# loop-Z/omniisaacgymenvs_loop

Measured on AMD Instinct MI355X. Metric: env-steps/sec USV_CaptureXY at 1/2/4/8 MI355X; wall-clock to reward=30, higher is better.
Workload: dtype fp32

## Files before the change

### omniisaacgymenvs_loop_amd/csrc/ppo.hip

```cpp
#include <cstdlib>
#include <cstring>
#include <type_traits>

#include "usv_device.h"

USV_PROBE_DEFINE(ppo)
USV_PROBE_DEFINE(pol)
USV_PROBE_DEFINE(red)

namespace {

constexpr int NIN = PPO_NIN, NH = PPO_NH, NA = PPO_NA;
constexpr int RB = 32;
constexpr int TB = 256;
constexpr int XS = 35;
constexpr int HS = 129;
constexpr int NPART = PPO_NPARAM + 8;
constexpr int NPART_PAD = (NPART + 3) & ~3;
constexpr int P_LOSS = PPO_NPARAM;
constexpr float kLog2Pi = 1.8378770664093453f;

typedef float f32x16 __attribute__((ext_vector_type(16)));
typedef unsigned int u32x4_t __attribute__((ext_vector_type(4)));

// ... 797 lines not shown
#pragma unroll
      for (int u = 0; u < 8; ++u) xv[u] = obs[(size_t)min(r0 + u * nl, bnd - 1) * NIN + col];
#pragma unroll
      for (int u = 0; u < 8; ++u)
        if (r0 + u * nl < bnd) {
          const double x = xv[u];
          s += x; s2 += x * x;
        }
    }
    acc[0][col][lane_r] = s;
    acc[1][col][lane_r] = s2;
  }
  __syncthreads();
  if (tid < NIN) {
    double t = 0, t2 = 0;
    for (int l = 0; l < nl; ++l) { t += acc[0][tid][l]; t2 += acc[1][tid][l]; }
    double *o = part + ((size_t)mb * OM_CH + ch) * 2 * NIN;
    o[tid] = t;
    o[NIN + tid] = t2;
  }
}

constexpr int RS_TB = 256, RS_U = 8;
__global__ __launch_bounds__(RS_TB) void k_obs_rms_seq(ppo_cfg_t c, const double *__restrict__ part, int nmb,
                                                       double *obs_rms, double *seq) {
  const double rows = (double)c.minibatch;
  for (int q = threadIdx.x; q < nmb * NIN; q += RS_TB) {
    const int mb = q / NIN, k = q % NIN;
    double sa = 0, sb = 0;
#pragma unroll
    for (int ch = 0; ch < OM_CH; ++ch) {
      const double *o = part + ((size_t)mb * OM_CH + ch) * 2 * NIN;
      sa += o[k];
      sb += o[NIN + k];
    }
    const double bmean = sa / rows;
    seq[(size_t)mb * 2 * NIN + k] = bmean;
    seq[(size_t)mb * 2 * NIN + NIN + k] = (sb - rows * bmean * bmean) / (rows - 1.0);
  }
  __syncthreads();
  const int k = threadIdx.x;
  if (k < NIN) {
    double mean = obs_rms[k], var = obs_rms[NIN + k], count = obs_rms[2 * NIN];
    for (int mb0 = 0; mb0 < nmb; mb0 += RS_U) {
      double bm[RS_U], bv[RS_U];
#pragma unroll
      for (int u = 0; u < RS_U; ++u) {
        const int mb = min(mb0 + u, nmb - 1);
        bm[u] = seq[(size_t)mb * 2 * NIN + k];
        bv[u] = seq[(size_t)mb * 2 * NIN + NIN + k];
      }
#pragma unroll
      for (int u = 0; u < RS_U; ++u) {
        if (mb0 + u >= nmb) break;
        const double tot = count + rows;
        const double delta = bm[u] - mean;
        const double M2 = var * count + bv[u] * rows + delta * delta * count * rows / tot;
        mean = mean + delta * rows / tot;
        var = M2 / tot;
        count = tot;
        seq[(size_t)(mb0 + u) * 2 * NIN + k] = mean;
        seq[(size_t)(mb0 + u) * 2 * NIN + NIN + k] = var;
      }
    }
    obs_rms[k] = mean;
    obs_rms[NIN + k] = var;
    if (k == 0) obs_rms[2 * NIN] = count;
  }
}

constexpr int GTB = 512;

#ifndef USV_RD_P
#define USV_RD_P 128
#endif
typedef float f32x4v __attribute__((ext_vector_type(4)));
constexpr int RD_TB = 512, RD_P = USV_RD_P;
constexpr int RD_L = RD_P / 4;
constexpr int RD_G = (RD_TB / RD_L);
constexpr int RD_KB = 16;
constexpr int RED_BLOCKS = (PPO_NPARAM + 5 + RD_P - 1) / RD_P;
static_assert(RD_P % 4 == 0 && 64 % RD_L == 0 && RD_P <= RD_TB, "reduce geometry");
static_assert(RED_BLOCKS <= 256, "chunk squares: one per thread of waves 0-3");
constexpr int W2IMG_FLOATS = (NH * HS + 3) & ~3;
constexpr int W2IMG_OFF = (PPO_NPARAM + 8 + RED_BLOCKS + 3) & ~3;
constexpr int W2IMG_PIECES = W2IMG_FLOATS / 256;
constexpr int W2IMG_LAST_LANES = W2IMG_FLOATS % 256 / 4;
static_assert(W2IMG_FLOATS == NH * HS && W2IMG_PIECES % 8 == 0 && W2IMG_LAST_LANES > 0 && W2IMG_LAST_LANES < 64,
              "W2 image: the copy covers s.w2 exactly, 8 waves x whole pieces + one partial piece");

struct AdamBanks {
  const float *P0, *m0, *v0;
  float *P1, *m1, *v1;
};
struct AdamK {
  float step_size, bc2s;
};
__device__ __forceinline__ AdamK adam_consts(const ppo_cfg_t &c, float lr, float step) {
  const double bc1 = 1.0 - pow((double)c.adam_b1, (double)step);
  const double bc2 = 1.0 - pow((double)c.adam_b2, (double)step);
  return {(float)((double)lr / bc1), (float)sqrt(bc2)};
}
__device__ __forceinline__ void adam_one(const ppo_cfg_t &c, const AdamK &k, float g, float p_old, float m_old,
                                         float v_old, float &pn, float &mn, float &vn) {
  if (c.weight_decay != 0.f) g = g + c.weight_decay * p_old;
  mn = m_old + (1.0f - c.adam_b1) * (g - m_old);
  vn = v_old * c.adam_b2 + (1.0f - c.adam_b2) * g * g;
  const float denom = sqrtf(vn) / k.bc2s + c.adam_eps;
  pn = p_old - k.step_size * (mn / denom);
}
__device__ __forceinline__ float clip_coef(const ppo_cfg_t &c, float total_norm) {
  float coef = 1.0f;
  if (c.truncate_grads) {
    coef = c.grad_norm / (total_norm + 1e-6f);
    coef = fminf(coef, 1.0f);
  }
  return coef;
}
__device__ __forceinline__ AdamK adam_consts_tagged(const ppo_cfg_t &c, float lr, float step, float t_ss,
                                                    float t_bc, float t_step, float t_lr) {
  if (t_step == step && t_lr == lr) return {t_ss, t_bc};
  return adam_consts(c, lr, step);
}
struct OptNext {
  float nl, kl_keep, step;
  AdamK nk;
};
template <class OptIn>
__device__ __forceinline__ OptNext opt_next(const ppo_cfg_t &c, const OptIn &opt_in, float kl) {
  const float lr = opt_in[0];
  float nl = lr, kl_keep = opt_in[2];
  if (c.lr_adaptive) {
    if (kl > 2.0f * c.kl_threshold) nl = fmaxf(lr / 1.5f, c.lr_min);
    if (kl < 0.5f * c.kl_threshold) nl = fminf(lr * 1.5f, c.lr_max);
    kl_keep = kl;
  }
  const float step = opt_in[1] + 1.0f;
  return {nl, kl_keep, step, adam_consts(c, nl, step + 1.0f)};
}
__device__ __forceinline__ void opt_store(const ppo_cfg_t &c, const OptNext &x, float *opt_out, float total_norm,
                                          float kl, float *kl_out) {
  if (c.lr_adaptive && kl_out) *kl_out = kl;
  opt_out[0] = x.nl;
  opt_out[1] = x.step;
  opt_out[2] = x.kl_keep;
  opt_out[3] = total_norm;
  opt_out[4] = x.nk.step_size;
  opt_out[5] = x.nk.bc2s;
  opt_out[6] = x.step + 1.0f;
  opt_out[7] = x.nl;
}

struct ChainIn {
  const float *P_prev, *m_prev, *v_prev;
  float *P_cur, *m_cur, *v_cur;
  const float *grad;
  const float *opt_prev;
  float *opt_cur;
  float *kl_out;
  uint32_t *dp_clock;
  int fold_skip;
  float gscale;
};

constexpr int XG = XS;
constexpr int GX = ((RB * XG + GTB - 1) / GTB) * GTB;
struct GradSmem {
  alignas(16) float w2[NH * HS];
  float w1[NH * XG];
  float x[GX];
  float h1[RB * HS];
  float h2[RB * HS];
  float xch[4][16][64];
  float out[RB * 4];
  float g[RB * 4];
  float hg[4][4][NH];
  float b1[NH];
  float tail[TAIL + 1];
  float nrm[4];
  int fold[2];
};

constexpr int S_W2 = 0, S_W1 = NH * NH, S_SIG = S_W1 + NH * 32, S_B1 = S_SIG + 2, S_TAIL = S_B1 + NH,
              S_W1C = S_TAIL + TAIL, S_END = S_W1C + NH;
static_assert(S_END == PPO_NPARAM && S_W1 % 4 == 0 && NIN == 33, "partial slot layout");
__device__ __forceinline__ int tail_slot(int param) { return S_TAIL + param - PPO_OFF_B2; }
__device__ __forceinline__ int acc_slot(int base, int tile, int a, int lane) { return base + ((tile * 4 + a) * 64 + lane) * 4; }
__device__ __forceinline__ int param_of_slot(int s) {
  if (s < S_W1) {
    const int tile = s >> 10, a = (s >> 8) & 3, lane = (s >> 2) & 63, q = 4 * a + (s & 3);
    const int n = 32 * (tile >> 2) + crow(q, lane >> 5), k = 32 * (tile & 3) + (lane & 31);
    return PPO_OFF_W2 + n * NH + k;
  }
  if (s < S_SIG) {
    const int t = s - S_W1, tile = t >> 10, a = (t >> 8) & 3, lane = (t >> 2) & 63, q = 4 * a + (t & 3);
    const int n = 32 * tile + crow(q, lane >> 5), k = lane & 31;
    return PPO_OFF_W1 + n * NIN + k;
  }
  if (s < S_B1) return PPO_OFF_SIGMA + (s - S_SIG);
  if (s < S_TAIL) return PPO_OFF_B1 + (s - S_B1);
  if (s < S_W1C) return PPO_OFF_B2 + (s - S_TAIL);
  if (s < S_END) return PPO_OFF_W1 + (s - S_W1C) * NIN + (NIN - 1);
  return -1;
}

struct RowIn {
  float act0, act1, nlp, val, ret, adv, mu0, mu1, sg0, sg1;
};

#ifndef USV_PART_AUX
#define USV_PART_AUX 2
#endif
template <int kAux, bool kCM>
struct PartOutT {
  __amdgpu_buffer_rsrc_t r;
  uint32_t cs;
  __device__ __forceinline__ uint32_t off(int idx) const {
    if constexpr (kCM) return (uint32_t)(idx / RD_P) * cs + (uint32_t)(idx % RD_P) * 4u;
    else return (uint32_t)idx * 4u;
  }
  __device__ __forceinline__ void operator()(int idx, float v) const {
    __builtin_amdgcn_raw_buffer_store_b32(__builtin_bit_cast(uint32_t, v), r, off(idx), 0, kAux);
  }
  __device__ __forceinline__ void x4(int idx, float a, float b, float c, float d) const {
    const u32x4_t v = {__builtin_bit_cast(uint32_t, a), __builtin_bit_cast(uint32_t, b), __builtin_bit_cast(uint32_t, c),
                       __builtin_bit_cast(uint32_t, d)};
    __builtin_amdgcn_raw_buffer_store_b128(v, r, off(idx), 0, kAux);
  }
};
constexpr int AUX_SC1 = 16;

constexpr int FOLD_G = 8;
static_assert(RD_G >= FOLD_G, "k_reduce_partials(fold = 1) reads one group row per row group");
constexpr int FOLD_MAX_M = 32;
constexpr int FOLD_CTL_STRIDE = 64;
constexpr uint64_t FOLD_WAIT_TICKS = 10000;
__host__ __device__ constexpr size_t part_body_floats(int nblk) {
  return (size_t)nblk * RED_BLOCKS * RD_P > (size_t)(nblk + FOLD_G) * NPART_PAD ? (size_t)nblk * RED_BLOCKS * RD_P
                                                                                 : (size_t)(nblk + FOLD_G) * NPART_PAD;
}
__device__ __forceinline__ uint32_t *fold_ctl(float *partials, int nblk) {
  return reinterpret_cast<uint32_t *>(partials + part_body_floats(nblk));
}
__device__ __forceinline__ const uint32_t *fold_ctl(const float *partials, int nblk) {
  return reinterpret_cast<const uint32_t *>(partials + part_body_floats(nblk));
}
__device__ __forceinline__ f32x4v ld4_sc1(__amdgpu_buffer_rsrc_t r, uint32_t byte_off) {
  return __builtin_bit_cast(f32x4v, __builtin_amdgcn_raw_buffer_load_b128(r, byte_off, 0, AUX_SC1));
}

__device__ __forceinline__ void lds_dma16(const float *src, uint32_t lds_dst) {
  uint32_t keep;
  __asm__ volatile("s_mov_b32 %0, m0\n\ts_mov_b32 m0, %2\n\ts_nop 0\n\tglobal_load_lds_dwordx4 %1, off\n\t"
                   "s_mov_b32 m0, %0"
                   : "=&s"(keep)
                   : "v"(src), "s"(lds_dst)
                   : "memory");
}

__device__ __forceinline__ void redo_step(const ppo_cfg_t &c, const ChainIn &ch, const float (&op)[8], float coef,
                                          float scale, GradSmem &s, float &ls0, float &ls1) {
  const AdamK ak = adam_consts_tagged(c, op[0], op[1] + 1.0f, op[4], op[5], op[6], op[7]);
  for (int q = threadIdx.x; q < PPO_NPARAM; q += GTB) {
    float pn, mn, vn;
    adam_one(c, ak, ch.grad[q] * scale * coef, ch.P_prev[q], ch.m_prev[q], ch.v_prev[q], pn, mn, vn);
    if ((q / GTB) % gridDim.x == blockIdx.x) {
      ch.P_cur[q] = pn; ch.m_cur[q] = mn; ch.v_cur[q] = vn;
    }
    if (q >= PPO_OFF_B2) {
      s.tail[q - PPO_OFF_B2] = pn;
    } else if (q >= PPO_OFF_W2) {
      const int e = q - PPO_OFF_W2;
      s.w2[(e / NH) * HS + e % NH] = pn;
    } else if (q >= PPO_OFF_B1) {
      s.b1[q - PPO_OFF_B1] = pn;
    } else if (q >= PPO_OFF_W1) {
      const int e = q - PPO_OFF_W1;
      s.w1[(e / NIN) * XG + e % NIN] = pn;
    }
  }
  float pn, mn, vn;
  adam_one(c, ak, ch.grad[PPO_OFF_SIGMA] * scale * coef, ch.P_prev[PPO_OFF_SIGMA], ch.m_prev[PPO_OFF_SIGMA],
           ch.v_prev[PPO_OFF_SIGMA], pn, mn, vn);
  ls0 = pn;
  adam_one(c, ak, ch.grad[PPO_OFF_SIGMA + 1] * scale * coef, ch.P_prev[PPO_OFF_SIGMA + 1],
           ch.m_prev[PPO_OFF_SIGMA + 1], ch.v_prev[PPO_OFF_SIGMA + 1], pn, mn, vn);
  ls1 = pn;
}

constexpr int APN_TB = 256;
__device__ __forceinline__ float apply_norm_part(const float *__restrict__ grad_in, float grad_scale, int tid) {
  constexpr int N4 = PPO_NPARAM / 4, U = (N4 + APN_TB - 1) / APN_TB;
  const float4 *g4 = reinterpret_cast<const float4 *>(grad_in);
  float4 gv[U];
#pragma unroll
  for (int u = 0; u < U; ++u) gv[u] = g4[min(tid + u * APN_TB, N4 - 1)];
  float ss = 0.f;
#pragma unroll
  for (int u = 0; u < U; ++u) {
    if (tid + u * APN_TB >= N4) continue;
    const float x = gv[u].x * grad_scale, y = gv[u].y * grad_scale;
    const float z = gv[u].z * grad_scale, w = gv[u].w * grad_scale;
    ss = fmaf(x, x, ss); ss = fmaf(y, y, ss); ss = fmaf(z, z, ss); ss = fmaf(w, w, ss);
  }
  for (int r = 4 * N4 + tid; r < PPO_NPARAM; r += APN_TB) {
    const float g = grad_in[r] * grad_scale;
    ss = fmaf(g, g, ss);
  }
  return ss;
}

template <bool kBf, bool kChain, bool kFold, bool kColl = false>
__device__ __forceinline__ void mb_grad8w(const ppo_cfg_t &c, const ChainIn &ch, const float *__restrict__ P,
                                          const double *__restrict__ obs_rms, int row0,
                                          const float *__restrict__ e_obs, const float *__restrict__ e_act,
                                          const float *__restrict__ e_nlp, const float *__restrict__ e_val,
                                          const float *__restrict__ e_ret, const float *__restrict__ e_adv,
                                          float *e_mu, float *e_sigma, float *partials, GradSmem &s) {
  const int tid = threadIdx.x, lane = tid & 63, w = tid >> 6;
  const int i = lane & 31, h = lane >> 5;
  const int kh = w >> 2, cb = w & 3, n0 = 32 * cb;
  const int rb0 = row0 + blockIdx.x * RB;
  const float invB = 1.0f / (float)c.minibatch;
  USV_PHASE(ppo, 0);
  if (ch.dp_clock && blockIdx.x == 0 && tid == 0) *ch.dp_clock += 1u;
  constexpr int NW1G = (NH * XG + GTB - 1) / GTB, NTLG = (TAIL + GTB - 1) / GTB, NW2F = NH * NH / GTB;
  static_assert(NH * NH % GTB == 0, "staging trip counts");
  constexpr bool kImg = kChain && !kColl && !kFold;
  float w2f[kImg ? 1 : NW2F];
  float w1r[NW1G], tlr[NTLG];
  float ov = 0.f;
  if constexpr (kChain) ov = lane < 8 ? ch.opt_prev[lane] : ch.grad[PPO_NPARAM];
  {
#pragma unroll
    for (int u = 0; u < NW1G; ++u) {
      const int q = min(tid + u * GTB, NH * XG - 1), j = q / XG, k = q % XG;
      w1r[u] = P[PPO_OFF_W1 + j * NIN + min(k, NIN - 1)];
    }
#pragma unroll
    for (int u = 0; u < NTLG; ++u) tlr[u] = P[PPO_OFF_B2 + min(tid + u * GTB, TAIL - 1)];
  }
  const float b1r = P[PPO_OFF_B1 + (tid & (NH - 1))];
  float lsv;
  if constexpr (!kImg) lsv = P[PPO_OFF_SIGMA + (lane & 1)];
  float lsig0 = 0.f, lsig1 = 0.f;
  float csq = 0.f;
  if constexpr (kChain) csq = ch.grad[PPO_NPARAM + 8 + min(tid, RED_BLOCKS - 1)];
  RowIn ri;
  const auto load_rows = [&] {
    const size_t row = (size_t)rb0 + (lane & (RB - 1));
    ri.act0 = e_act[row * 2]; ri.act1 = e_act[row * 2 + 1];
    ri.nlp = e_nlp[row]; ri.adv = e_adv[row];
    ri.val = e_val[row]; ri.ret = e_ret[row];
    ri.mu0 = e_mu[row * 2]; ri.mu1 = e_mu[row * 2 + 1];
    ri.sg0 = e_sigma[row * 2]; ri.sg1 = e_sigma[row * 2 + 1];
  };
  if constexpr (!kImg) load_rows();
  constexpr int NU = (RB * XG + GTB - 1) / GTB;
  float xo[NU];
  double mu[NU], var[NU];
#pragma unroll
  for (int u = 0; u < NU; ++u) {
    const int q = min(tid + u * GTB, RB * XG - 1), r = q / XG, kc = min(q % XG, NIN - 1);
    xo[u] = e_obs[(size_t)(rb0 + r) * NIN + kc];
    mu[u] = obs_rms[kc];
    var[u] = obs_rms[NIN + kc];
  }
  if constexpr (kImg) {
    lsv = P[PPO_OFF_SIGMA + (lane & 1)];
    load_rows();
    const int wu = __builtin_amdgcn_readfirstlane(w);
    const uint32_t w2lds = (uint32_t)(uintptr_t)(__attribute__((address_space(3))) float *)s.w2;
    const float *img = ch.grad + W2IMG_OFF + lane * 4;
    if (wu == GTB / 64 - 1 && lane < W2IMG_LAST_LANES)
      lds_dma16(img + W2IMG_PIECES * 256, w2lds + W2IMG_PIECES * 1024);
#pragma unroll
    for (int u = 0; u < W2IMG_PIECES / (GTB / 64); ++u) {
      const int pc = wu + (GTB / 64) * u;
      lds_dma16(img + pc * 256, w2lds + pc * 1024);
    }
  } else {
#pragma unroll
    for (int u = 0; u < NW2F; ++u) w2f[u] = P[PPO_OFF_W2 + tid + u * GTB];
  }
  __builtin_amdgcn_sched_barrier(0);
#pragma unroll
  for (int u = 0; u < NW1G; ++u)
    if ((tid + u * GTB) % XG >= NIN) w1r[u] = 0.f;
  if (kChain && tid >= RED_BLOCKS) csq = 0.f;
  {
    const bool norm = c.normalize_input != 0;
#pragma unroll
    for (int u = 0; u < NU; ++u) {
      const int q = tid + u * GTB;
      const int k = q % XG;
      const float xn = rms_norm(xo[u], mu[u], var[u], c.rms_eps);
      const float xv = (k < NIN && q < RB * XG) ? (norm ? xn : xo[u]) : 0.f;
      s.x[q] = xv;
    }
  }
#pragma unroll
  for (int u = 0; u < NW1G; ++u)
    if (tid + u * GTB < NH * XG) s.w1[tid + u * GTB] = w1r[u];
#pragma unroll
  for (int u = 0; u < NTLG; ++u)
    if (tid + u * GTB < TAIL) s.tail[tid + u * GTB] = tlr[u];
  if (tid < NH) s.b1[tid] = b1r;
  if (kChain && !kColl && w < 4) {
    const float t = wave_sum(csq);
    if (lane == 0) s.nrm[w] = t;
  }
  __syncthreads();
  if constexpr (kColl) {
    if (w < 4) {
      const float t = wave_sum(apply_norm_part(ch.grad, ch.gscale, tid));
      if (lane == 0) s.nrm[w] = t;
    }
    __syncthreads();
  }
  bool slow = false;
  if constexpr (kChain) {
    const auto lane_of = [&](int q) {
      return __builtin_bit_cast(float, __builtin_amdgcn_readlane(__builtin_bit_cast(int, ov), q));
    };
    const float total_norm = sqrtf(((s.nrm[0] + s.nrm[1]) + s.nrm[2]) + s.nrm[3]);
    const float coef = clip_coef(c, total_norm);
    const float gscale = kColl ? ch.gscale : 1.0f;
    if (blockIdx.x == 0 && tid == 256) {
      float op[8];
#pragma unroll
      for (int q = 0; q < 8; ++q) op[q] = lane_of(q);
      const float kl_prev = kColl ? lane_of(8) * gscale : lane_of(8);
      opt_store(c, opt_next(c, op, kl_prev), ch.opt_cur, total_norm, kl_prev, ch.kl_out);
    }
    if (kColl || coef < 1.0f) {
      slow = true;
      if constexpr (kImg) {
        __asm__ volatile("s_waitcnt vmcnt(0)" ::: "memory");
        __syncthreads();
      }
      float op[8];
#pragma unroll
      for (int q = 0; q < 8; ++q) op[q] = lane_of(q);
      redo_step(c, ch, op, coef, gscale, s, lsig0, lsig1);
      __syncthreads();
    }
  }
  USV_PHASE(ppo, 1);
  if (kh == 0) {
    f32x16 acc = {};
#pragma unroll
    for (int st = 0; st < 17; ++st) {
      const int k = 2 * st + h;
      acc = mfma32(s.x[i * XG + k], s.w1[(n0 + i) * XG + k], acc);
    }
    const float bj = s.b1[n0 + i];
#pragma unroll
    for (int r = 0; r < 16; ++r) s.h1[crow(r, h) * HS + n0 + i] = fast_tanh(acc[r] + bj);
  }
  USV_PHASE(ppo, 9);
  if constexpr (kImg) {
    __asm__ volatile("s_waitcnt vmcnt(0)" ::: "memory");
  } else if (!slow) {
#pragma unroll
    for (int u = 0; u < NW2F; ++u) {
      const int e = tid + u * GTB;
      s.w2[(e >> 7) * HS + (e & (NH - 1))] = w2f[u];
    }
  }
  __syncthreads();
  USV_PHASE(ppo, 10);
  const int ra = (i + 16 * kh) & (RB - 1);
  {
    f32x16 acc = {};
    if constexpr (kBf) {
#pragma unroll
      for (int st = 0; st < NH / 32; ++st) {
        const int k0 = 64 * kh + 16 * st + 8 * h;
        acc = mfma_bf16(ld8(&s.h1[ra * HS + k0]), ld8(&s.w2[(n0 + i) * HS + k0]), acc);
      }
    } else {
#pragma unroll 16
      for (int st = 0; st < NH / 4; ++st) {
        const int k = 64 * kh + 2 * st + h;
        acc = mfma32(s.h1[ra * HS + k], s.w2[(n0 + i) * HS + k], acc);
      }
    }
    USV_PHASE(ppo, 11);
#pragma unroll
    for (int q = 0; q < 8; ++q) s.xch[cb][8 * kh + q][lane] = acc[8 + q];
// ... 346 lines not shown
    for (int r = 0; r < dp.world; ++r) st_sys(dp_x(dp.peer[r], par, dp.rank) + slot, pv);
  __asm__ volatile("s_waitcnt vmcnt(0)" ::: "memory");
  __syncthreads();
  if (w == 0) {
    if (lane < dp.world) {
      if constexpr ((USV_DP_ORDER & 1) != 0) {
        __builtin_amdgcn_fence(__ATOMIC_RELEASE, "");
        __asm__ volatile("s_waitcnt vmcnt(0)" ::: "memory");
        __hip_atomic_store(dp_flag(dp.peer[lane], chunk, dp.rank), key, __ATOMIC_RELAXED, __HIP_MEMORY_SCOPE_SYSTEM);
      } else {
        __hip_atomic_store(dp_flag(dp.peer[lane], chunk, dp.rank), key, __ATOMIC_RELAXED, __HIP_MEMORY_SCOPE_SYSTEM);
      }
    }
    const uint64_t t0 = wall_clock64(), lim = (uint64_t)timeout_ms * 100000ull;
    bool got = lane >= dp.world;
    while (true) {
      if (!got) {
        const uint32_t f = __hip_atomic_load(dp_flag(dp.peer[dp.rank], chunk, lane), __ATOMIC_RELAXED,
                                             __HIP_MEMORY_SCOPE_SYSTEM);
        got = (int32_t)(f - key) >= 0;
      }
      if (__all(got)) break;
      const int32_t e = __hip_atomic_load(dp.err, __ATOMIC_RELAXED, __HIP_MEMORY_SCOPE_AGENT);
      if (e != 0) break;
      if (wall_clock64() - t0 > lim) {
        if (lane == 0) atomicOr(dp.err, 1);
        break;
      }
      __builtin_amdgcn_s_sleep(2);
    }
    if constexpr ((USV_DP_ORDER & 2) != 0) {
      __builtin_amdgcn_fence(__ATOMIC_ACQUIRE, "");
      __asm__ volatile("s_waitcnt vmcnt(0)" ::: "memory");
    }
  }
  __syncthreads();
  float t = 0.f;
  if (tid < RD_P) {
    const float *xs = dp_x(dp.peer[dp.rank], par, 0);
    for (int r = 0; r < dp.world; ++r) t += ld_sys(xs + (size_t)r * DP_SLOTS + slot);
  }
  return t;
}

__device__ __forceinline__ float dp_probe_value(int sender, int round, int slot) {
  return (float)(sender * 1000003 + round * 65537 + slot);
}
__global__ __launch_bounds__(RD_TB) void k_dp_selftest(ppo_dp_t dp, uint32_t key0, int rounds, int timeout_ms) {
  const int tid = threadIdx.x;
  const int slot = blockIdx.x * RD_P + tid;
  for (int rd = 0; rd < rounds; ++rd) {
    const uint32_t key = key0 + (uint32_t)rd;
    (void)dp_exchange(dp, key, blockIdx.x, slot, dp_probe_value(dp.rank, rd, slot & 0xffff), timeout_ms);
    if (tid < RD_P) {
      const float *xs = dp_x(dp.peer[dp.rank], (int)(key & 1u), 0);
      bool bad = false;
      for (int r = 0; r < dp.world; ++r)
        bad |= ld_sys(xs + (size_t)r * DP_SLOTS + slot) != dp_probe_value(r, rd, slot & 0xffff);
      if (bad) atomicOr(dp.err, 2);
    }
    __syncthreads();
  }
}

template <bool kSpec, bool kDP>
__global__ __launch_bounds__(RD_TB) void k_reduce_partials(const float *__restrict__ partials, int nblk, float *grad,
                                                           float *losses, float inv_b, ppo_cfg_t c, AdamBanks a,
                                                           const float *__restrict__ opt_in, ppo_dp_t dp, int fold) {
  __shared__ float4 red[RD_G][RD_L];
  __shared__ float sqw[RD_TB / 64];
  USV_PHASE(red, 0);
  const int tid = threadIdx.x, lane = tid & 63, w = tid >> 6;
  const int col = tid % RD_L, grp = tid / RD_L;
  const int p4 = blockIdx.x * RD_L + col;
  const bool ok = p4 < NPART_PAD / 4;
  const float4 *P4 = reinterpret_cast<const float4 *>(partials);
  const int myslot = blockIdx.x * RD_P + tid;
  const bool mine = kSpec && tid < RD_P && myslot < S_END;
  const int pq = mine ? param_of_slot(myslot) : 0;
  float p_old = 0.f, m_old = 0.f, v_old = 0.f;
  if (mine) {
    p_old = a.P0[pq]; m_old = a.m0[pq]; v_old = a.v0[pq];
  }
  uint32_t key = 0u;
  if (kDP) key = *dp.clock;
  float4 acc = make_float4(0.f, 0.f, 0.f, 0.f);
  float oin[8] = {};
  if (kSpec) {
#pragma unroll
    for (int q = 0; q < 8; ++q) oin[q] = opt_in[q];
  }
  const int p4c = min(p4, NPART_PAD / 4 - 1);
  if (fold) {
    if (grp < FOLD_G) {
      const int M = nblk / FOLD_G;
      const uint32_t *ctl = fold_ctl(partials, nblk) + grp * FOLD_CTL_STRIDE;
      const uint32_t gen = ctl[0] / (uint32_t)M;
      bool folded = true;
      for (int mm = 0; mm < M; ++mm) folded &= ctl[32 + mm] == gen;
      if (folded) {
        acc = P4[(size_t)(nblk + grp) * (NPART_PAD / 4) + p4c];
      } else {
        const int h0 = (M + 1) / 2;
        float4 a0 = make_float4(0.f, 0.f, 0.f, 0.f), a1 = a0;
        for (int mm = 0; mm < M; ++mm) {
          const float4 x = P4[(size_t)(grp + FOLD_G * mm) * (NPART_PAD / 4) + p4c];
          float4 &t = mm < h0 ? a0 : a1;
          t.x += x.x; t.y += x.y; t.z += x.z; t.w += x.w;
        }
        acc = make_float4(a0.x + a1.x, a0.y + a1.y, a0.z + a1.z, a0.w + a1.w);
      }
    }
  } else
  for (int b0 = grp; b0 < nblk; b0 += RD_G * RD_KB) {
    float4 x[RD_KB];
#pragma unroll
    for (int k = 0; k < RD_KB; ++k) {
      const int row = min(b0 + RD_G * k, nblk - 1);
      const float4 *src = P4 + ((size_t)blockIdx.x * nblk + row) * RD_L + col;
      const f32x4v v = __builtin_nontemporal_load(reinterpret_cast<const f32x4v *>(src));
      x[k] = make_float4(v[0], v[1], v[2], v[3]);
    }
#pragma unroll
    for (int k = 0; k < RD_KB; ++k) {
      if (ok && b0 + RD_G * k < nblk) {
        acc.x += x[k].x; acc.y += x[k].y; acc.z += x[k].z; acc.w += x[k].w;
      }
    }
  }
  USV_PHASE(red, 1);
  AdamK ak = {0.f, 1.f};
  if (kSpec)
    ak = adam_consts_tagged(c, oin[0], oin[1] + 1.0f, oin[4], oin[5], oin[6], oin[7]);
  red[grp][col] = acc;
  __syncthreads();
  float s = 0.f;
  const int slot = blockIdx.x * RD_P + tid;
  if (tid < RD_P) {
#pragma unroll
    for (int g = 0; g < RD_G; ++g) s += reinterpret_cast<const float *>(red[g])[tid];
  }
  USV_PHASE(red, 2);
  float sl = s;
  if constexpr (kDP) {
    const float pv = slot < S_END ? s : (slot == PPO_NPARAM + 4 ? s * inv_b : 0.f);
    s = dp_exchange(dp, key, blockIdx.x, slot, pv, dp.timeout_ms) / (float)dp.world;
  }
  float sq = 0.f;
  if (tid < RD_P) {
    if (slot < S_END) {
      grad[param_of_slot(slot)] = s;
      sq = s * s;
      if (mine) {
        float pn, mn, vn;
        adam_one(c, ak, s, p_old, m_old, v_old, pn, mn, vn);
        a.P1[pq] = pn; a.m1[pq] = mn; a.v1[pq] = vn;
        if (pq >= PPO_OFF_W2 && pq < PPO_OFF_B2) {
          const int e = pq - PPO_OFF_W2;
          grad[W2IMG_OFF + (e / NH) * HS + e % NH] = pn;
        }
      }
    } else if (slot < PPO_NPARAM + 5) {
      const int q = slot - PPO_NPARAM;
      if (q == 4) grad[PPO_NPARAM] = kDP ? s : s * inv_b;
      if (losses) losses[q] = sl * inv_b;
    }
  }
  USV_PHASE(red, 3);
  if (w < (RD_P + 63) / 64) {
    sq = wave_sum(sq);
    if (lane == 0) sqw[w] = sq;
  }
  __syncthreads();
  if (tid == 0) {
    float t = 0.f;
#pragma unroll
    for (int q = 0; q < (RD_P + 63) / 64; ++q) t += sqw[q];
    grad[PPO_NPARAM + 8 + blockIdx.x] = t;
  }
  USV_PHASE(red, 4);
}

constexpr int AP_TB = 256;
template <bool kNormFromPartials, bool kFinish>
__global__ __launch_bounds__(AP_TB) void k_apply(ppo_cfg_t c, AdamBanks a, const float *__restrict__ grad_in,
                                                 const float *__restrict__ opt_in, float *__restrict__ opt_out,
                                                 float grad_scale, float *kl_out) {
  __shared__ float red[AP_TB / 64];
  const int tid = threadIdx.x;
  const int q = blockIdx.x * AP_TB + tid;
  const int qc = min(q, PPO_NPARAM - 1);
  const float g_raw = grad_in[qc], p_old = a.P0[qc], m_old = a.m0[qc], v_old = a.v0[qc];
  const float s0 = grad_in[PPO_NPARAM + 8 + min(tid, RED_BLOCKS - 1)];
  const float lr = opt_in[0];
  const float step = opt_in[1] + 1.0f;
  const float kl = grad_in[PPO_NPARAM] * grad_scale;
  __builtin_amdgcn_sched_barrier(0);
  const AdamK ak = adam_consts_tagged(c, lr, step, opt_in[4], opt_in[5], opt_in[6], opt_in[7]);
  OptNext nx = {};
  if (blockIdx.x == 0 && tid == 0) nx = opt_next(c, opt_in, kl);
  __asm__ volatile("" : : "v"(ak.step_size), "v"(ak.bc2s), "v"(nx.nl), "v"(nx.nk.step_size), "v"(nx.nk.bc2s));
  float ss = 0.f;
  if (kNormFromPartials) {
    ss = tid < RED_BLOCKS ? s0 : 0.f;
  } else {
    constexpr int N4 = PPO_NPARAM / 4, U = (N4 + AP_TB - 1) / AP_TB;
    const float4 *g4 = reinterpret_cast<const float4 *>(grad_in);
    float4 gv[U];
#pragma unroll
    for (int u = 0; u < U; ++u) gv[u] = g4[min(tid + u * AP_TB, N4 - 1)];
#pragma unroll
    for (int u = 0; u < U; ++u) {
      if (tid + u * AP_TB >= N4) continue;
      const float x = gv[u].x * grad_scale, y = gv[u].y * grad_scale;
      const float z = gv[u].z * grad_scale, w = gv[u].w * grad_scale;
      ss = fmaf(x, x, ss); ss = fmaf(y, y, ss); ss = fmaf(z, z, ss); ss = fmaf(w, w, ss);
    }
    for (int r = 4 * N4 + tid; r < PPO_NPARAM; r += AP_TB) {
      const float g = grad_in[r] * grad_scale;
      ss = fmaf(g, g, ss);
    }
  }
  ss = wave_sum(ss);
  if ((tid & 63) == 0) red[tid >> 6] = ss;
  __syncthreads();
  const float total_norm = sqrtf(((red[0] + red[1]) + red[2]) + red[3]);
  const float coef = clip_coef(c, total_norm);
  if (q < PPO_NPARAM && (!kFinish || coef < 1.0f)) {
    float pn, mn, vn;
    adam_one(c, ak, g_raw * grad_scale * coef, p_old, m_old, v_old, pn, mn, vn);
    a.P1[q] = pn;
    a.m1[q] = mn;
    a.v1[q] = vn;
  }
  if (blockIdx.x == 0 && tid == 0) opt_store(c, nx, opt_out, total_norm, kl, kl_out);
}

}

extern "C" {

int ppo_policy_step(const ppo_cfg_t *cfg, const float *params, const double *obs_rms, const double *val_rms,
// ... 349 lines not shown
```

### omniisaacgymenvs_loop_amd/csrc/usv_device.h

```cpp
#pragma once
#include <hip/hip_runtime.h>
#include <stdint.h>
#include "../../include/usv_hip.h"

#define USV_PI_F 3.14159265358979323846f
#define USV_2PI_F 6.28318530717958647692f

struct u32x4 { uint32_t x, y, z, w; };

__device__ __forceinline__ u32x4 philox4x32_10(u32x4 c, uint32_t k0, uint32_t k1) {
#pragma unroll
  for (int r = 0; r < 10; ++r) {
    const uint32_t lo0 = 0xD2511F53u * c.x, hi0 = __umulhi(0xD2511F53u, c.x);
    const uint32_t lo1 = 0xCD9E8D57u * c.z, hi1 = __umulhi(0xCD9E8D57u, c.z);
    c = u32x4{hi1 ^ c.y ^ k0, lo1, hi0 ^ c.w ^ k1, lo0};
    k0 += 0x9E3779B9u;
    k1 += 0xBB67AE85u;
  }
  return c;
}

__device__ __forceinline__ float u01(uint32_t x) { return (float)(x >> 8) * (1.0f / 16777216.0f); }

__device__ __forceinline__ void philox_u4(uint64_t seed, uint32_t env, uint64_t step, uint32_t site_blk,
// ... 194 lines not shown
  const int lane = threadIdx.x & 63, o = lane & 15, q = lane >> 4, gbase = lane & 48;
  auto Ue = [&](int i) -> float {
    if (inj) return inj[(size_t)ee * USV_NU_RESET + i];
    float u4[4];
    philox_u4(seed, (uint32_t)ee, step, 0x100u + (uint32_t)(i >> 2), u4);
    return u4[i & 3];
  };
  const float mnx = tx - c.obst_box, mny = ty - c.obst_box;
  const float dx_ = (tx + c.obst_box) - mnx, dy_ = (ty + c.obst_box) - mny;
  float ox = Ue(RU_OBST + 2 * o) * dx_ + mnx;
  float oy = Ue(RU_OBST + 2 * o + 1) * dy_ + mny;
  const float sep2 = c.min_obs_sep * c.min_obs_sep;
  bool done = false;
  for (int r = 0; !done; ++r) {
    const int itq = 4 * r + q;
    float cx = 0.f, cy = 0.f;
    if (itq < USV_SPAWN_ITERS) {
      const int rb = RU_RESAMPLE + itq * USV_NOBST * 2;
      cx = Ue(rb + 2 * o) * dx_ + mnx;
      cy = Ue(rb + 2 * o + 1) * dy_ + mny;
    }
    for (int qq = 0; qq < 4; ++qq) {
      const int it = 4 * r + qq;
      const float ds = tnorm2(ox - sx, oy - sy);
      const float dt = tnorm2(ox - tx, oy - ty);
      const bool vo = ox < 900.f;
      bool bad = q == 0 && ((ds < c.min_dist_safe) || (dt < c.min_dist_safe));
#pragma unroll
      for (int k = 0; k < 4; ++k) {
        const int i = 4 * q + k;
        const float xi = __shfl(ox, gbase + i, 64), yi = __shfl(oy, gbase + i, 64);
        const float ddx = xi - ox, ddy = yi - oy;
        if (i < o && vo && (xi < 900.f) && (ddx * ddx + ddy * ddy) < sep2) bad = true;
      }
      const uint64_t bq = __ballot(bad);
      const uint32_t inval = (uint32_t)((bq | (bq >> 16) | (bq >> 32) | (bq >> 48)) & 0xFFFFull);
      bad = ((inval >> o) & 1u) != 0u;
      if (inval == 0) { done = true; break; }
      if (it == USV_SPAWN_ITERS) {
        if (bad) { ox = 999.0f; oy = 999.0f; }
        done = true;
        break;
      }
      const float nx = __shfl(cx, 16 * qq + o, 64), ny = __shfl(cy, 16 * qq + o, 64);
      if (bad) { ox = nx; oy = ny; }
    }
  }
  (void)q;
  return make_float2(ox, oy);
}


__device__ __forceinline__ float wave_sum(float v) {
#pragma unroll
  for (int off = 32; off > 0; off >>= 1) v += __shfl_xor(v, off, 64);
  return v;
}
__device__ __forceinline__ float wave_max(float v) {
#pragma unroll
  for (int off = 32; off > 0; off >>= 1) v = fmaxf(v, __shfl_xor(v, off, 64));
  return v;
}
__device__ __forceinline__ float wave_min(float v) {
#pragma unroll
  for (int off = 32; off > 0; off >>= 1) v = fminf(v, __shfl_xor(v, off, 64));
  return v;
}

__device__ __forceinline__ void nan_report(int32_t *flag, uint32_t bits) {
  if (__ballot(bits != 0u) == 0ull) return;
  uint32_t m = bits;
#pragma unroll
  for (int off = 32; off > 0; off >>= 1) m |= (uint32_t)__shfl_xor((int)m, off, 64);
  if ((threadIdx.x & 63) == 0) atomicOr(flag, (int)m);
}
__device__ __forceinline__ uint32_t nonfinite(float x) { return isfinite(x) ? 0u : 1u; }

__device__ __forceinline__ void atomic_max_f32(float *addr, float v) {
  if (v >= 0.f) atomicMax((int *)addr, __float_as_int(v));
  else atomicMin((unsigned int *)addr, __float_as_uint(v));
}

#ifdef USV_PHASE_PROBE
#define USV_PROBE_DEFINE(tu)                                                           \
  __device__ unsigned long long g_probe_##tu[4096][16];                                \
  extern "C" int usv_probe_read_##tu(void *host_out) {                                 \
    return (int)hipMemcpyFromSymbol(host_out, HIP_SYMBOL(g_probe_##tu), sizeof(g_probe_##tu)); \
  }
#define USV_PHASE(tu, k)                                                               \
  do {                                                                                 \
    if (threadIdx.x == 0 && blockIdx.x < 4096) g_probe_##tu[blockIdx.x][k] = wall_clock64(); \
  } while (0)
#define USV_PHASE_T(tu, k, t)                                                          \
  do {                                                                                 \
    if (threadIdx.x == (t) && blockIdx.x < 4096) g_probe_##tu[blockIdx.x][k] = wall_clock64(); \
  } while (0)
#define USV_PHASE_DRAIN(tu, k, t)                                                      \
  do {                                                                                 \
    __asm__ volatile("s_waitcnt vmcnt(0)" ::: "memory");                               \
    USV_PHASE_T(tu, k, t);                                                             \
  } while (0)
#else
#define USV_PROBE_DEFINE(tu)
#define USV_PHASE(tu, k) ((void)0)
#define USV_PHASE_T(tu, k, t) ((void)0)
#define USV_PHASE_DRAIN(tu, k, t) ((void)0)
#endif

#define USV_CHECK_LAUNCH()                                   \
  do {                                                       \
    hipError_t _e = hipGetLastError();                       \
    if (_e != hipSuccess) return 100 + (int)_e;              \
  } while (0)
```

Measured before the change: 36.36 million.

## Stage W1, b1 and tail weights via Adam-written LDS image with DMA

The Adam step now writes padded copies of W1 (row stride XS with zeroed pads), b1 and the output tail into a contiguous image in the grad buffer, laid out to match GradSmem w1|b1|tail. The chained grad kernel copies that image straight into LDS with 16-byte direct-to-LDS DMA, replacing per-thread register staging and scalar LDS stores. Observation staging is also reworked so each thread holds one fixed column, loading obs_rms mean and variance once instead of per pass, with float normalization. The cost is extra global writes in Adam, a larger grad buffer, added probe instrumentation, and a tighter layout coupling enforced by static asserts.

```diff
diff --git a/omniisaacgymenvs_loop_amd/csrc/ppo.hip b/omniisaacgymenvs_loop_amd/csrc/ppo.hip
--- a/omniisaacgymenvs_loop_amd/csrc/ppo.hip
+++ b/omniisaacgymenvs_loop_amd/csrc/ppo.hip
@@ -903,8 +903,12 @@
 constexpr int RED_BLOCKS = (PPO_NPARAM + 5 + RD_P - 1) / RD_P;
 static_assert(RD_P % 4 == 0 && 64 % RD_L == 0 && RD_P <= RD_TB, "reduce geometry");
 static_assert(RED_BLOCKS <= 256, "chunk squares: one per thread of waves 0-3");
+constexpr int WIMG_B1 = NH * XS, WIMG_TAIL = WIMG_B1 + NH, WIMG_FLOATS = (WIMG_TAIL + TAIL + 3) & ~3;
+constexpr int WIMG_OFF = (PPO_NPARAM + 8 + RED_BLOCKS + 3) & ~3;
+constexpr int WIMG_PIECES = WIMG_FLOATS / 256, WIMG_LAST_LANES = WIMG_FLOATS % 256 / 4;
+static_assert(WIMG_B1 % 4 == 0 && WIMG_LAST_LANES > 0 && WIMG_LAST_LANES < 64, "weight image: 16-byte pieces");
 constexpr int W2IMG_FLOATS = (NH * HS + 3) & ~3;
-constexpr int W2IMG_OFF = (PPO_NPARAM + 8 + RED_BLOCKS + 3) & ~3;
+constexpr int W2IMG_OFF = WIMG_OFF + WIMG_FLOATS;
 constexpr int W2IMG_PIECES = W2IMG_FLOATS / 256;
 constexpr int W2IMG_LAST_LANES = W2IMG_FLOATS % 256 / 4;
 static_assert(W2IMG_FLOATS == NH * HS && W2IMG_PIECES % 8 == 0 && W2IMG_LAST_LANES > 0 && W2IMG_LAST_LANES < 64,
@@ -985,10 +989,14 @@
 };
 
 constexpr int XG = XS;
-constexpr int GX = ((RB * XG + GTB - 1) / GTB) * GTB;
+constexpr int XRP = GTB / XG, XPT = XRP * XG, NXU = (RB + XRP - 1) / XRP;
+constexpr int GX = NXU * XPT + (GTB - XPT);
+static_assert(GX >= RB * XG && XPT <= GTB, "obs staging passes");
 struct GradSmem {
   alignas(16) float w2[NH * HS];
-  float w1[NH * XG];
+  alignas(16) float w1[NH * XG];
+  float b1[NH];
+  float tail[TAIL + 1];
   float x[GX];
   float h1[RB * HS];
   float h2[RB * HS];
@@ -996,11 +1004,13 @@
   float out[RB * 4];
   float g[RB * 4];
   float hg[4][4][NH];
-  float b1[NH];
-  float tail[TAIL + 1];
   float nrm[4];
   int fold[2];
 };
+static_assert(offsetof(GradSmem, w1) % 16 == 0 && offsetof(GradSmem, b1) == offsetof(GradSmem, w1) + WIMG_B1 * 4 &&
+                  offsetof(GradSmem, tail) == offsetof(GradSmem, w1) + WIMG_TAIL * 4 &&
+                  sizeof(GradSmem::tail) >= (WIMG_FLOATS - WIMG_TAIL) * 4,
+              "the image's first region lands on w1 | b1 | tail as one flat copy");
 
 constexpr int S_W2 = 0, S_W1 = NH * NH, S_SIG = S_W1 + NH * 32, S_B1 = S_SIG + 2, S_TAIL = S_B1 + NH,
               S_W1C = S_TAIL + TAIL, S_END = S_W1C + NH;
@@ -1149,10 +1159,23 @@
   static_assert(NH * NH % GTB == 0, "staging trip counts");
   constexpr bool kImg = kChain && !kColl && !kFold;
   float w2f[kImg ? 1 : NW2F];
-  float w1r[NW1G], tlr[NTLG];
+  float w1r[kImg ? 1 : NW1G], tlr[kImg ? 1 : NTLG], b1r = 0.f;
+  if constexpr (kImg) {
+    const int wu = __builtin_amdgcn_readfirstlane(w);
+    const uint32_t w1lds = (uint32_t)(uintptr_t)(__attribute__((address_space(3))) float *)s.w1;
+    const float *img = ch.grad + WIMG_OFF + lane * 4;
+    if (wu == GTB / 64 - 1 && lane < WIMG_LAST_LANES)
+      lds_dma16(img + WIMG_PIECES * 256, w1lds + WIMG_PIECES * 1024);
+#pragma unroll
+    for (int u = 0; u < (WIMG_PIECES + GTB / 64 - 1) / (GTB / 64); ++u) {
+      const int pc = wu + (GTB / 64) * u;
+      if ((GTB / 64) * (u + 1) <= WIMG_PIECES || pc < WIMG_PIECES)
+        lds_dma16(img + pc * 256, w1lds + pc * 1024);
+    }
+  }
   float ov = 0.f;
   if constexpr (kChain) ov = lane < 8 ? ch.opt_prev[lane] : ch.grad[PPO_NPARAM];
-  {
+  if constexpr (!kImg) {
 #pragma unroll
     for (int u = 0; u < NW1G; ++u) {
       const int q = min(tid + u * GTB, NH * XG - 1), j = q / XG, k = q % XG;
@@ -1160,8 +1183,8 @@
     }
 #pragma unroll
     for (int u = 0; u < NTLG; ++u) tlr[u] = P[PPO_OFF_B2 + min(tid + u * GTB, TAIL - 1)];
-  }
-  const float b1r = P[PPO_OFF_B1 + (tid & (NH - 1))];
+    b1r = P[PPO_OFF_B1 + (tid & (NH - 1))];
+  }
   float lsv;
   if constexpr (!kImg) lsv = P[PPO_OFF_SIGMA + (lane & 1)];
   float lsig0 = 0.f, lsig1 = 0.f;
@@ -1177,16 +1200,11 @@
     ri.sg0 = e_sigma[row * 2]; ri.sg1 = e_sigma[row * 2 + 1];
   };
   if constexpr (!kImg) load_rows();
-  constexpr int NU = (RB * XG + GTB - 1) / GTB;
-  float xo[NU];
-  double mu[NU], var[NU];
-#pragma unroll
-  for (int u = 0; u < NU; ++u) {
-    const int q = min(tid + u * GTB, RB * XG - 1), r = q / XG, kc = min(q % XG, NIN - 1);
-    xo[u] = e_obs[(size_t)(rb0 + r) * NIN + kc];
-    mu[u] = obs_rms[kc];
-    var[u] = obs_rms[NIN + kc];
-  }
+  const int xk = tid % XG, xr = tid / XG, xkc = min(xk, NIN - 1);
+  const double omu = obs_rms[xkc], ovar = obs_rms[NIN + xkc];
+  float xo[NXU];
+#pragma unroll
+  for (int u = 0; u < NXU; ++u) xo[u] = e_obs[(size_t)(rb0 + min(xr + u * XRP, RB - 1)) * NIN + xkc];
   if constexpr (kImg) {
     lsv = P[PPO_OFF_SIGMA + (lane & 1)];
     load_rows();
@@ -1205,28 +1223,34 @@
     for (int u = 0; u < NW2F; ++u) w2f[u] = P[PPO_OFF_W2 + tid + u * GTB];
   }
   __builtin_amdgcn_sched_barrier(0);
-#pragma unroll
-  for (int u = 0; u < NW1G; ++u)
-    if ((tid + u * GTB) % XG >= NIN) w1r[u] = 0.f;
+  USV_PHASE(ppo, 16);
+  if constexpr (!kImg) {
+#pragma unroll
+    for (int u = 0; u < NW1G; ++u)
+      if ((tid + u * GTB) % XG >= NIN) w1r[u] = 0.f;
+  }
   if (kChain && tid >= RED_BLOCKS) csq = 0.f;
+  const float om = (float)omu, od = sqrtf((float)ovar + c.rms_eps);
+  USV_PHASE_LANDED(ppo, 17, xo[NXU - 1]);
   {
     const bool norm = c.normalize_input != 0;
 #pragma unroll
-    for (int u = 0; u < NU; ++u) {
-      const int q = tid + u * GTB;
-      const int k = q % XG;
-      const float xn = rms_norm(xo[u], mu[u], var[u], c.rms_eps);
-      const float xv = (k < NIN && q < RB * XG) ? (norm ? xn : xo[u]) : 0.f;
-      s.x[q] = xv;
-    }
-  }
-#pragma unroll
-  for (int u = 0; u < NW1G; ++u)
-    if (tid + u * GTB < NH * XG) s.w1[tid + u * GTB] = w1r[u];
-#pragma unroll
-  for (int u = 0; u < NTLG; ++u)
-    if (tid + u * GTB < TAIL) s.tail[tid + u * GTB] = tlr[u];
-  if (tid < NH) s.b1[tid] = b1r;
+    for (int u = 0; u < NXU; ++u) {
+      const float xn = clampt((xo[u] - om) / od, -5.0f, 5.0f);
+      const float xv = xk < NIN ? (norm ? xn : xo[u]) : 0.f;
+      s.x[tid < XPT ? tid + u * XPT : NXU * XPT + (tid - XPT)] = xv;
+    }
+  }
+  if constexpr (!kImg) {
+#pragma unroll
+    for (int u = 0; u < NW1G; ++u)
+      if (tid + u * GTB < NH * XG) s.w1[tid + u * GTB] = w1r[u];
+#pragma unroll
+    for (int u = 0; u < NTLG; ++u)
+      if (tid + u * GTB < TAIL) s.tail[tid + u * GTB] = tlr[u];
+    if (tid < NH) s.b1[tid] = b1r;
+  }
+  USV_PHASE(ppo, 18);
   if (kChain && !kColl && w < 4) {
     const float t = wave_sum(csq);
     if (lane == 0) s.nrm[w] = t;
@@ -1739,6 +1763,22 @@
   if (mine) {
     p_old = a.P0[pq]; m_old = a.m0[pq]; v_old = a.v0[pq];
   }
+  int iq = -1;
+  bool zpad = false;
+  if (mine) {
+    if (pq >= PPO_OFF_B2) {
+      iq = WIMG_OFF + WIMG_TAIL + (pq - PPO_OFF_B2);
+    } else if (pq >= PPO_OFF_W2) {
+      const int e = pq - PPO_OFF_W2;
+      iq = W2IMG_OFF + (e / NH) * HS + e % NH;
+    } else if (pq >= PPO_OFF_B1) {
+      iq = WIMG_OFF + WIMG_B1 + (pq - PPO_OFF_B1);
+    } else if (pq >= PPO_OFF_W1) {
+      const int e = pq - PPO_OFF_W1, k = e % NIN;
+      iq = WIMG_OFF + (e / NIN) * XS + k;
+      zpad = k == NIN - 1;
+    }
+  }
   uint32_t key = 0u;
   if (kDP) key = *dp.clock;
   float4 acc = make_float4(0.f, 0.f, 0.f, 0.f);
@@ -1812,9 +1852,9 @@
         float pn, mn, vn;
         adam_one(c, ak, s, p_old, m_old, v_old, pn, mn, vn);
         a.P1[pq] = pn; a.m1[pq] = mn; a.v1[pq] = vn;
-        if (pq >= PPO_OFF_W2 && pq < PPO_OFF_B2) {
-          const int e = pq - PPO_OFF_W2;
-          grad[W2IMG_OFF + (e / NH) * HS + e % NH] = pn;
+        if (iq >= 0) grad[iq] = pn;
+        if (zpad) {
+          grad[iq + 1] = 0.f; grad[iq + 2] = 0.f;
         }
       }
     } else if (slot < PPO_NPARAM + 5) {
diff --git a/omniisaacgymenvs_loop_amd/csrc/usv_device.h b/omniisaacgymenvs_loop_amd/csrc/usv_device.h
--- a/omniisaacgymenvs_loop_amd/csrc/usv_device.h
+++ b/omniisaacgymenvs_loop_amd/csrc/usv_device.h
@@ -300,8 +300,9 @@
 }
 
 #ifdef USV_PHASE_PROBE
+#define USV_PROBE_SLOTS 24
 #define USV_PROBE_DEFINE(tu)                                                           \
-  __device__ unsigned long long g_probe_##tu[4096][16];                                \
+  __device__ unsigned long long g_probe_##tu[4096][USV_PROBE_SLOTS];                   \
   extern "C" int usv_probe_read_##tu(void *host_out) {                                 \
     return (int)hipMemcpyFromSymbol(host_out, HIP_SYMBOL(g_probe_##tu), sizeof(g_probe_##tu)); \
   }
@@ -318,9 +319,15 @@
     __asm__ volatile("s_waitcnt vmcnt(0)" ::: "memory");                               \
     USV_PHASE_T(tu, k, t);                                                             \
   } while (0)
+#define USV_PHASE_LANDED(tu, k, v)                                                     \
+  do {                                                                                 \
+    __asm__ volatile("" ::"v"(v));                                                     \
+    USV_PHASE(tu, k);                                                                  \
+  } while (0)
 #else
 #define USV_PROBE_DEFINE(tu)
 #define USV_PHASE(tu, k) ((void)0)
+#define USV_PHASE_LANDED(tu, k, v) ((void)0)
 #define USV_PHASE_T(tu, k, t) ((void)0)
 #define USV_PHASE_DRAIN(tu, k, t) ((void)0)
 #endif
```

Result: slower. 35.70 million (-1.8%).
